# latticeboltzmann/2d-lb

Hardware: AMD Instinct MI355X
Metric: MLUPS (million lattice updates per second), fused D2Q9 BGK step (higher is better)
Workload: dtype f32

## Files before the change

2d-lb_amd/csrc/kernels_deep.h:

```cpp
#pragma once

#ifdef LB_DIAG
#define LB_DEEP_NOCOLLIDE if (!(a.diag & 1))
#else
#define LB_DEEP_NOCOLLIDE
#endif

namespace {

constexpr int DEEP_RW = 1, DEEP_PFD = 1;
constexpr int DEEP_WSLOTS = 8;
constexpr bool deep_pairs(bool mask, int bc) { return !mask && bc == LB_BC_PERIODIC; }

template <int RW, int NL>
struct DeepState {
    Window w[RW > 0 ? RW : 1];
    f4a d0[NL];
    unsigned mhist;
};
typedef unsigned u4v __attribute__((ext_vector_type(4)));
struct DeepCtx {
    int lane, x4, ym, n_iter;
    bool store_lane;
    f4a (*mine)[64], (*other)[64];
    f4a (*ho)[64];
    f4a (*dma)[64];
    unsigned dma_off;
};
constexpr int DEEP_WHOLE = 0, DEEP_FRONT = 1, DEEP_BACK = 2;
constexpr int DEEP_HO_SLOTS = 10;

__device__ __forceinline__ void deep_window_load(f4a (*W)[64], int lane, int it, f4a d0, Window &w)
{
    const int gs = 2 + 3 * (it & 1);
    w.d0 = d0; w.d1 = W[0][lane]; w.d3 = W[1][lane];
    w.g2 = W[gs][lane]; w.g5 = W[gs + 1][lane]; w.g6 = W[gs + 2][lane];
}
template <bool DOWN>
__device__ __forceinline__ void deep_window_push(f4a (*W)[64], int lane, int it, f4a &d0, const f4a (&q)[9])
{
    typedef Dir<DOWN> D_;
    const int gs = 2 + 3 * (it & 1);
    d0 = q[0]; W[0][lane] = q[1]; W[1][lane] = q[3];
    W[gs][lane] = q[D_::A]; W[gs + 1][lane] = q[D_::B]; W[gs + 2][lane] = q[D_::C];
}
template <bool DOWN>
__device__ __forceinline__ void deep_publish(f4a (*W)[64], int lane, int gs, const f4a (&q)[9])
{
    typedef Dir<DOWN> D_;
    W[gs][lane] = q[D_::An]; W[gs + 1][lane] = q[D_::Bn]; W[gs + 2][lane] = q[D_::Cn];
}

constexpr int DEEP_NUM_RECORDS = -1;
__device__ __forceinline__ float *deep_uniform(const float *p)
{
    const unsigned long long v = (unsigned long long)p;
    const unsigned lo = __builtin_amdgcn_readfirstlane((unsigned)v), hi = __builtin_amdgcn_readfirstlane((unsigned)(v >> 32));
    return reinterpret_cast<float *>(((unsigned long long)hi << 32) | lo);
}
__device__ __forceinline__ f4a deep_buf_load(__amdgpu_buffer_rsrc_t r, int vo, int so, int imm)
{
    return __builtin_bit_cast(f4a, __builtin_amdgcn_raw_buffer_load_b128(r, vo + imm, so, 0));
}
template <int BC, bool MASK>
__device__ __forceinline__ void deep_row_load(const StepArgs &a, int r, int x4, Row1 &o)
{
    int ym, yp;
    o.have = step1_rows(a, r, o.rr, ym, yp);
    o.mk = uc4{0, 0, 0, 0};
    o.hsolid = false;
    o.hxc = -1;
    if (o.have) {
        const long long P = a.pitch, S = a.plane;
        const float *s = a.src;
        const int yl = o.rr;
        o.wp = WrapPatch{0.f, 0.f, 0.f, 0.f, 0.f, 0.f};
        if (BC == LB_BC_PERIODIC) {
            const int c = a.nx - 1 - x4;
            const bool wrap_w = x4 == 0, wrap_e = c >= 0 && c < 4;
            if (wrap_w) {
                o.wp.p1 = s[1 * S + (long long)yl * P + a.nx - 1];
                o.wp.p5 = s[5 * S + (long long)ym * P + a.nx - 1];
                o.wp.p8 = s[8 * S + (long long)yp * P + a.nx - 1];
            }
            if (wrap_e) {
                o.wp.w3 = s[3 * S + (long long)yl * P];
                o.wp.w6 = s[6 * S + (long long)ym * P];
                o.wp.w7 = s[7 * S + (long long)yp * P];
            }
        }
        const __amdgpu_buffer_rsrc_t r0 = __builtin_amdgcn_make_buffer_rsrc(deep_uniform(s + (long long)yl * P - 1), 0, DEEP_NUM_RECORDS, 0x00020000);
        const __amdgpu_buffer_rsrc_t rm = __builtin_amdgcn_make_buffer_rsrc(deep_uniform(s + (long long)ym * P - 1), 0, DEEP_NUM_RECORDS, 0x00020000);
        const __amdgpu_buffer_rsrc_t rp = __builtin_amdgcn_make_buffer_rsrc(deep_uniform(s + (long long)yp * P - 1), 0, DEEP_NUM_RECORDS, 0x00020000);
        const unsigned S4 = (unsigned)a.plane * 4u;
        const int vo = x4 * 4;
        o.q[0] = deep_buf_load(r0, vo, 0, 4);
        o.q[1] = deep_buf_load(r0, vo, (int)(S4), 0);
        o.q[2] = deep_buf_load(rm, vo, (int)(2u * S4), 4);
        o.q[3] = deep_buf_load(r0, vo, (int)(3u * S4), 8);
        o.q[4] = deep_buf_load(rp, vo, (int)(4u * S4), 4);
        o.q[5] = deep_buf_load(rm, vo, (int)(5u * S4), 0);
        o.q[6] = deep_buf_load(rm, vo, (int)(6u * S4), 8);
        o.q[7] = deep_buf_load(rp, vo, (int)(7u * S4), 8);
        o.q[8] = deep_buf_load(rp, vo, (int)(8u * S4), 0);
        if (MASK) o.mk = *reinterpret_cast<const uc4 *>(lane_ptr(a.mask + (long long)yl * a.fpitch, x4));
    } else {
        o.wp = WrapPatch{0.f, 0.f, 0.f, 0.f, 0.f, 0.f};
#pragma unroll
        for (int k = 0; k < 9; ++k) o.q[k] = f4a{0.f, 0.f, 0.f, 0.f};
    }
}
#ifdef LB_DIAG
constexpr bool DEEP_MANUAL = false;
#else
constexpr bool DEEP_MANUAL = true;
#endif
__device__ __forceinline__ u4v deep_rsrc_words(const float *p)
{
    const unsigned long long v = (unsigned long long)p;
    return u4v{(unsigned)__builtin_amdgcn_readfirstlane((unsigned)v), (unsigned)__builtin_amdgcn_readfirstlane((unsigned)(v >> 32)), (unsigned)DEEP_NUM_RECORDS,
               0x00020000u};
}
template <int BC, bool MASK>
__device__ __forceinline__ void deep_row_issue(const StepArgs &a, int r, int x4, Row1 &o)
{
    int ym, yp;
    o.have = step1_rows(a, r, o.rr, ym, yp);
    o.hsolid = false;
    o.hxc = -1;
    if (o.have) {
        const long long P = a.pitch, S = a.plane;
        const float *s = a.src;
        const int yl = o.rr;
        if (BC == LB_BC_PERIODIC) {
            const int c = a.nx - 1 - x4;
            const bool wrap_w = x4 == 0, wrap_e = c >= 0 && c < 4;
            if (wrap_w) {
                const float *e = s + a.nx - 1;
                asm volatile("global_load_dword a36, %0, off\n\tglobal_load_dword a37, %1, off\n\tglobal_load_dword a38, %2, off"
                             :: "v"(e + 1 * S + (long long)yl * P), "v"(e + 5 * S + (long long)ym * P), "v"(e + 8 * S + (long long)yp * P)
                             : "memory", "a36", "a37", "a38");
            }
            if (wrap_e) {
                asm volatile("global_load_dword a39, %0, off\n\tglobal_load_dword a40, %1, off\n\tglobal_load_dword a41, %2, off"
                             :: "v"(s + 3 * S + (long long)yl * P), "v"(s + 6 * S + (long long)ym * P), "v"(s + 7 * S + (long long)yp * P)
                             : "memory", "a39", "a40", "a41");
            }
        }
        const u4v r0 = deep_rsrc_words(s + (long long)yl * P - 1), rm = deep_rsrc_words(s + (long long)ym * P - 1),
                  rp = deep_rsrc_words(s + (long long)yp * P - 1);
        const unsigned S4 = (unsigned)a.plane * 4u;
        asm volatile("buffer_load_dwordx4 a[0:3], %0, %1, 0 offen offset:4\n\t"
                     "buffer_load_dwordx4 a[4:7], %0, %1, %4 offen\n\t"
                     "buffer_load_dwordx4 a[8:11], %0, %2, %5 offen offset:4\n\t"
                     "buffer_load_dwordx4 a[12:15], %0, %1, %6 offen offset:8\n\t"
                     "buffer_load_dwordx4 a[16:19], %0, %3, %7 offen offset:4\n\t"
                     "buffer_load_dwordx4 a[20:23], %0, %2, %8 offen\n\t"
                     "buffer_load_dwordx4 a[24:27], %0, %2, %9 offen offset:8\n\t"
                     "buffer_load_dwordx4 a[28:31], %0, %3, %10 offen offset:8\n\t"
                     "buffer_load_dwordx4 a[32:35], %0, %3, %11 offen"
                     :: "v"(x4 * 4), "s"(r0), "s"(rm), "s"(rp), "s"(S4), "s"(2u * S4), "s"(3u * S4), "s"(4u * S4), "s"(5u * S4), "s"(6u * S4),
                        "s"(7u * S4), "s"(8u * S4)
                     : "memory", "a0", "a1", "a2", "a3", "a4", "a5", "a6", "a7", "a8", "a9", "a10", "a11", "a12", "a13",
                       "a14", "a15", "a16", "a17", "a18", "a19", "a20", "a21", "a22", "a23", "a24", "a25", "a26", "a27", "a28",
                       "a29", "a30", "a31", "a32", "a33", "a34", "a35");
        if (MASK) asm volatile("global_load_dword a42, %0, off" :: "v"(lane_ptr(a.mask + (long long)yl * a.fpitch, x4)) : "memory", "a42");
    }
}
template <int BC, bool MASK, int N>
__device__ __forceinline__ void deep_row_take(Row1 &o)
{
    static_assert(N == 0 || N == 9 || N == 12, "the stores of one steady iteration, or nothing");
#define LB_DEEP_TAKE_OUTS "={a[0:3]}"(o.q[0]), "={a[4:7]}"(o.q[1]), "={a[8:11]}"(o.q[2]), "={a[12:15]}"(o.q[3]), \
                          "={a[16:19]}"(o.q[4]), "={a[20:23]}"(o.q[5]), "={a[24:27]}"(o.q[6]), "={a[28:31]}"(o.q[7]), "={a[32:35]}"(o.q[8])
    if (N == 0) asm volatile("s_waitcnt vmcnt(0)" : LB_DEEP_TAKE_OUTS :: "memory");
    else if (N == 9) asm volatile("s_waitcnt vmcnt(9)" : LB_DEEP_TAKE_OUTS :: "memory");
    else asm volatile("s_waitcnt vmcnt(12)" : LB_DEEP_TAKE_OUTS :: "memory");
#undef LB_DEEP_TAKE_OUTS
    o.wp = WrapPatch{0.f, 0.f, 0.f, 0.f, 0.f, 0.f};
    if (BC == LB_BC_PERIODIC)
        asm volatile("" : "={a36}"(o.wp.p1), "={a37}"(o.wp.p5), "={a38}"(o.wp.p8), "={a39}"(o.wp.w3), "={a40}"(o.wp.w6), "={a41}"(o.wp.w7));
    o.mk = uc4{0, 0, 0, 0};
    if (MASK) {
        unsigned m;
        asm volatile("" : "={a42}"(m));
        o.mk = __builtin_bit_cast(uc4, m);
    }
    if (!o.have) {
#pragma unroll
        for (int k = 0; k < 9; ++k) o.q[k] = f4a{0.f, 0.f, 0.f, 0.f};
        o.mk = uc4{0, 0, 0, 0};
    }
}

template <int BC, bool MASK>
__device__ __forceinline__ void deep_row_issue_lds(const StepArgs &a, int r, int x4, unsigned slot, Row1 &o)
{
    int ym, yp;
    o.have = step1_rows(a, r, o.rr, ym, yp);
    o.hsolid = false;
    o.hxc = -1;
    if (o.have) {
        const long long P = a.pitch, S = a.plane;
        const float *s = a.src;
        const int yl = o.rr;
        unsigned m0_kept;
        asm volatile("s_waitcnt lgkmcnt(0)" ::: "memory");
        if (BC == LB_BC_PERIODIC) {
            const int c = a.nx - 1 - x4;
            const bool wrap_w = x4 == 0, wrap_e = c >= 0 && c < 4;
            if (wrap_w) {
                const float *e = s + a.nx - 1;
                asm volatile("s_mov_b32 %0, m0\n\ts_mov_b32 m0, %4\n\ts_nop 0\n\tglobal_load_lds_dword %1, off\n\t"
                             "s_add_u32 m0, m0, 0x100\n\ts_nop 0\n\tglobal_load_lds_dword %2, off\n\t"
                             "s_add_u32 m0, m0, 0x100\n\ts_nop 0\n\tglobal_load_lds_dword %3, off\n\ts_mov_b32 m0, %0"
                             : "=&s"(m0_kept)
                             : "v"(e + 1 * S + (long long)yl * P), "v"(e + 5 * S + (long long)ym * P), "v"(e + 8 * S + (long long)yp * P),
                               "s"(slot + 9 * 1024 + 256)
                             : "memory", "scc");
            }
            if (wrap_e) {
                asm volatile("s_mov_b32 %0, m0\n\ts_mov_b32 m0, %4\n\ts_nop 0\n\tglobal_load_lds_dword %1, off\n\t"
                             "s_add_u32 m0, m0, 0x100\n\ts_nop 0\n\tglobal_load_lds_dword %2, off\n\t"
                             "s_add_u32 m0, m0, 0x100\n\ts_nop 0\n\tglobal_load_lds_dword %3, off\n\ts_mov_b32 m0, %0"
                             : "=&s"(m0_kept)
                             : "v"(s + 3 * S + (long long)yl * P), "v"(s + 6 * S + (long long)ym * P), "v"(s + 7 * S + (long long)yp * P),
                               "s"(slot + 9 * 1024 + 256)
                             : "memory", "scc");
            }
        }
        const u4v r0 = deep_rsrc_words(s + (long long)yl * P - 1), rm = deep_rsrc_words(s + (long long)ym * P - 1),
                  rp = deep_rsrc_words(s + (long long)yp * P - 1);
        const unsigned S4 = (unsigned)a.plane * 4u;
        const int v0 = x4 * 4, v4 = v0 + 4, v8 = v0 + 8;
        asm volatile("s_mov_b32 %0, m0\n\ts_mov_b32 m0, %15\n\ts_nop 0\n\tbuffer_load_dwordx4 %2, %4, 0 offen lds\n\t"
                     "s_add_u32 m0, m0, 0x400\n\ts_nop 0\n\tbuffer_load_dwordx4 %1, %4, %7 offen lds\n\t"
                     "s_add_u32 m0, m0, 0x400\n\ts_nop 0\n\tbuffer_load_dwordx4 %2, %5, %8 offen lds\n\t"
                     "s_add_u32 m0, m0, 0x400\n\ts_nop 0\n\tbuffer_load_dwordx4 %3, %4, %9 offen lds\n\t"
                     "s_add_u32 m0, m0, 0x400\n\ts_nop 0\n\tbuffer_load_dwordx4 %2, %6, %10 offen lds\n\t"
                     "s_add_u32 m0, m0, 0x400\n\ts_nop 0\n\tbuffer_load_dwordx4 %1, %5, %11 offen lds\n\t"
                     "s_add_u32 m0, m0, 0x400\n\ts_nop 0\n\tbuffer_load_dwordx4 %3, %5, %12 offen lds\n\t"
                     "s_add_u32 m0, m0, 0x400\n\ts_nop 0\n\tbuffer_load_dwordx4 %3, %6, %13 offen lds\n\t"
                     "s_add_u32 m0, m0, 0x400\n\ts_nop 0\n\tbuffer_load_dwordx4 %1, %6, %14 offen lds\n\ts_mov_b32 m0, %0"
                     : "=&s"(m0_kept)
                     : "v"(v0), "v"(v4), "v"(v8), "s"(r0), "s"(rm), "s"(rp), "s"(S4), "s"(2u * S4), "s"(3u * S4), "s"(4u * S4), "s"(5u * S4),
                       "s"(6u * S4), "s"(7u * S4), "s"(8u * S4), "s"(slot)
                     : "memory", "scc");
        if (MASK)
            asm volatile("s_mov_b32 %0, m0\n\ts_mov_b32 m0, %2\n\ts_nop 0\n\tglobal_load_lds_dword %1, off\n\ts_mov_b32 m0, %0"
                         : "=&s"(m0_kept) : "v"(lane_ptr(a.mask + (long long)yl * a.fpitch, x4)), "s"(slot + 9 * 1024) : "memory");
    }
}
template <int BC, bool MASK>
__device__ __forceinline__ void deep_row_take_lds(const f4a (*S)[64], int lane, Row1 &o)
{
    asm volatile("s_waitcnt vmcnt(0)" ::: "memory");
    if (o.have) {
#pragma unroll
        for (int k = 0; k < 9; ++k) o.q[k] = S[k][lane];
        const unsigned *X = reinterpret_cast<const unsigned *>(S[9]);
        o.mk = MASK ? __builtin_bit_cast(uc4, X[lane]) : uc4{0, 0, 0, 0};
        o.wp = WrapPatch{0.f, 0.f, 0.f, 0.f, 0.f, 0.f};
        if (BC == LB_BC_PERIODIC) {
            const float e1 = __builtin_bit_cast(float, X[64 + lane]), e2 = __builtin_bit_cast(float, X[128 + lane]),
                        e3 = __builtin_bit_cast(float, X[192 + lane]);
            o.wp = WrapPatch{e1, e2, e3, e1, e2, e3};
        }
    } else {
        o.wp = WrapPatch{0.f, 0.f, 0.f, 0.f, 0.f, 0.f};
#pragma unroll
        for (int k = 0; k < 9; ++k) o.q[k] = f4a{0.f, 0.f, 0.f, 0.f};
        o.mk = uc4{0, 0, 0, 0};
    }
}

__device__ __forceinline__ void deep_row_store(const StepArgs &a, int r, int x4, const f4a (&t)[9])
{
    const __amdgpu_buffer_rsrc_t rd = __builtin_amdgcn_make_buffer_rsrc(deep_uniform(a.dst + (long long)r * a.pitch), 0, DEEP_NUM_RECORDS, 0x00020000);
    const unsigned S4 = (unsigned)a.plane * 4u;
    const int vo = x4 * 4;
    asm volatile("" ::: "memory");
    if (a.nts != 0) {
#pragma unroll
        for (int k = 0; k < 9; ++k) __builtin_amdgcn_raw_buffer_store_b128(__builtin_bit_cast(u4v, t[k]), rd, vo, (int)(k * S4), 2);
    } else {
#pragma unroll
        for (int k = 0; k < 9; ++k) __builtin_amdgcn_raw_buffer_store_b128(__builtin_bit_cast(u4v, t[k]), rd, vo, (int)(k * S4), 0);
    }
}

template <int BC, bool MASK, bool MACRO, int D, int RW, bool DOWN, int NST, int S, int ROLE = DEEP_WHOLE>
__device__ __forceinline__ void deep_stage(const StepArgs &a, const DeepCtx &cx, const int i, const int it,
                                           DeepState<RW, D - 1 - RW> &st, f4a (&qin)[9], f4a &r4, f4a &u4, f4a &v4)
{
    if constexpr (S <= D) {
        constexpr int K = S - 1;
        const int lane = cx.lane, x4 = cx.x4;
        constexpr int L = K > RW ? K - RW - 1 : 0;
        f4a (*W)[64] = cx.mine + L * DEEP_WSLOTS;
        if constexpr (NST >= S) {
            int r, t0_, t1_;
            (void)step1_rows(a, DOWN ? cx.ym - 1 - (i - K) : cx.ym + (i - K), r, t0_, t1_);
            f4a t[9];
            if constexpr (K <= RW) {
                skirt_gather<DOWN>(st.w[K - 1], qin, t);
                window_push_dir<DOWN>(st.w[K - 1], qin);
            } else {
                Window w;
                deep_window_load(W, lane, it, st.d0[L], w);
                skirt_gather<DOWN>(w, qin, t);
                deep_window_push<DOWN>(W, lane, it, st.d0[L], qin);
            }
            LB_DEEP_NOCOLLIDE collide_row<BC, MASK, true>(a, x4, a.y0 + r, t, mask_bits(st.mhist, K), r4, u4, v4);
            if constexpr (S == D && ROLE == DEEP_FRONT) {
#pragma unroll
                for (int k = 0; k < 9; ++k) cx.ho[k][lane] = t[k];
                if (MASK) reinterpret_cast<unsigned *>(cx.ho[9])[lane] = __builtin_bit_cast(unsigned, mask_bits(st.mhist, K));
            } else if constexpr (S == D) {
#ifdef LB_DIAG
                if (!(a.diag & (1 << 22)))
#endif
                if (cx.store_lane) {
                    deep_row_store(a, r, x4, t);
                    if (MACRO) {
                        const long long m = (long long)r * a.fpitch;
                        store_moments(a, m, x4, r4, u4, v4);
                    }
                }
            } else {
                if constexpr (NST == S) {
                    if constexpr (S <= RW) deep_publish<DOWN>(cx.other + (D - 2 - RW) * DEEP_WSLOTS, lane, S == 1 ? 5 : 2, t);
                    else deep_publish<DOWN>(cx.other + (S - RW - 1) * DEEP_WSLOTS, lane, 2 + 3 * (S & 1), t);
                }
                deep_stage<BC, MASK, MACRO, D, RW, DOWN, NST, S + 1, ROLE>(a, cx, i, it, st, t, r4, u4, v4);
            }
        } else if constexpr (NST == S - 1) {
            if constexpr (K <= RW) window_push_dir<DOWN>(st.w[K - 1], qin);
            else deep_window_push<DOWN>(W, lane, it, st.d0[L], qin);
        }
    }
}

template <int BC, bool MASK, bool MACRO, int D, int RW, int PFD, bool DOWN, int NST, int PAR = -1, int ROLE = DEEP_WHOLE>
__device__ __forceinline__ void deep_iter(const StepArgs &a, const DeepCtx &cx, const int i_, DeepState<RW, D - 1 - RW> &st, Row1 &cur,
                                          Row1 &nxt)
{
    static_assert(RW >= 0 && RW <= 2 && D - 1 - RW >= 1 && (ROLE == DEEP_WHOLE ? D - 2 > RW : D - 2 >= RW),
                  "register windows hand over through the last LDS window while it is idle");
    static_assert((D - 1 - RW) * DEEP_WSLOTS <= 40, "a wave has 40 KB of LDS at four waves per CU");
    const int lane = cx.lane, x4 = cx.x4;
    const int i = NST < D ? NST - 1 : i_;
    const int it = PAR >= 0 ? PAR : i;
    auto row_at = [&](int p) { return DOWN ? cx.ym - 1 - p : cx.ym + p; };
    f4a (*MB)[64] = cx.mine + (D - 2 - RW) * DEEP_WSLOTS;
    if (RW >= 1 && NST == 2) { st.w[0].g2 = MB[5][lane]; st.w[0].g5 = MB[6][lane]; st.w[0].g6 = MB[7][lane]; }
    if (RW >= 2 && NST == 3) { st.w[RW >= 2 ? 1 : 0].g2 = MB[2][lane]; st.w[RW >= 2 ? 1 : 0].g5 = MB[3][lane]; st.w[RW >= 2 ? 1 : 0].g6 = MB[4][lane]; }
#ifdef LB_DIAG
    if (!((a.diag & (1 << 23)) && i > 0))
#endif
    if constexpr (ROLE != DEEP_BACK) {
        if (ROLE == DEEP_FRONT) {
            deep_row_take_lds<BC, MASK>(cx.dma, lane, cur);
            deep_row_issue_lds<BC, MASK>(a, row_at(min(i + 1, cx.n_iter - 1)), x4, cx.dma_off, nxt);
        } else if (PFD && DEEP_MANUAL) {
            deep_row_take<BC, MASK, (NST < D ? 0 : (MACRO ? 12 : 9))>(cur);
            deep_row_issue<BC, MASK>(a, row_at(min(i + 1, cx.n_iter - 1)), x4, nxt);
        } else {
            static_assert(PFD == 1 || ROLE == DEEP_BACK, "a march that gathers its rows gathers them one ahead");
            deep_row_load<BC, MASK>(a, row_at(min(i + 1, cx.n_iter - 1)), x4, nxt);
        }
    }
    f4a (&q1)[9] = cur.q;
    f4a r4, u4, v4;
    const uc4 mk = cur.mk;
    if (ROLE != DEEP_BACK && cur.have) {
        gather_merge<BC, true>(a, x4, q1, cur.wp);
        LB_DEEP_NOCOLLIDE collide_row<BC, MASK, true>(a, x4, a.y0 + cur.rr, q1, mk, r4, u4, v4);
    }
    if (NST == 1) {
        if constexpr (RW >= 1) deep_publish<DOWN>(cx.other + (D - 2 - RW) * DEEP_WSLOTS, lane, 5, q1);
        else deep_publish<DOWN>(cx.other, lane, 2 + 3 * 1, q1);
    }
    deep_stage<BC, MASK, MACRO, D, RW, DOWN, NST, 2, ROLE>(a, cx, i, it, st, q1, r4, u4, v4);
    if (MASK) st.mhist = ((st.mhist | mask_word(mk)) << 1) & (0x01010101u * (unsigned)(((1 << D) - 2) & 0xff));
    if (ROLE == DEEP_WHOLE && NST < D) __syncthreads();
}

template <int BC, bool MASK, bool MACRO, int D, int RW, int PFD, bool DOWN, int NST>
__device__ __forceinline__ void deep_fill(const StepArgs &a, const DeepCtx &cx, DeepState<RW, D - 1 - RW> &st, Row1 &ra, Row1 &rb)
{
    if constexpr (NST < D) {
        if ((NST & 1) == 0) deep_iter<BC, MASK, MACRO, D, RW, PFD, DOWN, NST>(a, cx, NST - 1, st, rb, ra);
        else deep_iter<BC, MASK, MACRO, D, RW, PFD, DOWN, NST>(a, cx, NST - 1, st, ra, rb);
        deep_fill<BC, MASK, MACRO, D, RW, PFD, DOWN, NST + 1>(a, cx, st, ra, rb);
    }
}

template <int BC, bool MASK, bool MACRO, int D, int RW, int PFD, bool DOWN>
__device__ __forceinline__ void deep_march(const StepArgs &a, const int x0, const int ym, const int len, f4a (*mine)[64],
                                           f4a (*other)[64])
{
    DeepCtx cx;
    cx.lane = threadIdx.x;
    const int xr = x0 + cx.lane * 4;
    cx.x4 = skirt_column<BC>(a, xr, deep_skirt_lanes(D));
    cx.store_lane = skirt_store_lane(a, cx.lane, xr, deep_skirt_lanes(D));
    cx.ym = ym; cx.n_iter = len + D - 1;
    cx.mine = mine; cx.other = other;
    DeepState<RW, D - 1 - RW> st = {};
    auto row_at = [&](int p) { return DOWN ? ym - 1 - p : ym + p; };
    static_assert(PFD == 1, "a whole march gathers one row ahead");
    Row1 ra, rb;
    if (DEEP_MANUAL) deep_row_issue<BC, MASK>(a, row_at(0), cx.x4, ra);
    else deep_row_load<BC, MASK>(a, row_at(0), cx.x4, ra);
    deep_fill<BC, MASK, MACRO, D, RW, PFD, DOWN, 1>(a, cx, st, ra, rb);
    if (DEEP_MANUAL) asm volatile("s_waitcnt vmcnt(0)" ::: "memory");
    if (!deep_pairs(MASK, BC)) {
        if ((D - 1) & 1) ra = rb;
        for (int i = D - 1; i < cx.n_iter; ++i) {
            deep_iter<BC, MASK, MACRO, D, RW, PFD, DOWN, D>(a, cx, i, st, ra, rb);
            ra = rb;
        }
    } else {
        constexpr int P0 = (D - 1) & 1;
        int i = D - 1;
        for (; i + 1 < cx.n_iter; i += 2) {
            deep_iter<BC, MASK, MACRO, D, RW, PFD, DOWN, D, P0>(a, cx, i, st, P0 ? rb : ra, P0 ? ra : rb);
            deep_iter<BC, MASK, MACRO, D, RW, PFD, DOWN, D, 1 - P0>(a, cx, i + 1, st, P0 ? ra : rb, P0 ? rb : ra);
        }
        if (i < cx.n_iter) deep_iter<BC, MASK, MACRO, D, RW, PFD, DOWN, D, P0>(a, cx, i, st, P0 ? rb : ra, P0 ? ra : rb);
    }
    if (DEEP_MANUAL) asm volatile("s_waitcnt vmcnt(0)" ::: "memory");
}

template <int BC, bool MASK, bool MACRO, int D, int RW, int PFD>
__global__ __launch_bounds__(64 * STEP4_WAVES, PFD ? 1 : 2) void k_deep(const StepArgs a, int strips, int seg_rows, int nsegs, int row_end)
{
    __shared__ f4a lds_win[STEP4_WAVES][(D - 1 - RW) * DEEP_WSLOTS][64];
    const int wy = __builtin_amdgcn_readfirstlane(threadIdx.y);
    const int item = xcd_item(blockIdx.x, gridDim.x);
#ifdef LB_DIAG
    const unsigned long long diag_t0 = __builtin_amdgcn_s_memrealtime();
#endif
    int sx, sy;
    if (item < strips * nsegs) {
        sx = item % strips;
        sy = item / strips;
    } else {
        if (!a.edge_seg_rows) return;
        const int j = item - strips * nsegs;
        sx = (j & 1) ? strips - 1 : 0;
        sy = nsegs + (j >> 1);
    }
    int stride = a.seg_stride;
    if (a.edge_seg_rows && (sx == 0 || sx == strips - 1)) stride = seg_rows = a.edge_seg_rows;
    const int ya = a.row_begin + sy * stride;
    if (ya >= row_end) return;
    const int yb = min(ya + seg_rows, row_end);
    const int ym = ya + (yb - ya) / 2;
    const int x0 = sx * deep_valid(D) - 4 * deep_skirt_lanes(D);
    if (wy == 0) deep_march<BC, MASK, MACRO, D, RW, PFD, true>(a, x0, ym, ym - ya, lds_win[0], lds_win[1]);
    else deep_march<BC, MASK, MACRO, D, RW, PFD, false>(a, x0, ym, yb - ym, lds_win[1], lds_win[0]);
#ifdef LB_DIAG
    if ((a.diag & 4096) && threadIdx.x == 0) {
        __builtin_amdgcn_s_waitcnt(0);
        const unsigned long long t1 = __builtin_amdgcn_s_memrealtime();
        unsigned *o = reinterpret_cast<unsigned *>(a.rho) + 8 * (item * STEP4_WAVES + wy);
        o[0] = (unsigned)diag_t0; o[1] = (unsigned)(diag_t0 >> 32); o[2] = (unsigned)t1; o[3] = (unsigned)(t1 >> 32);
        o[4] = __builtin_amdgcn_s_getreg((31 << 11) | 20);
        o[5] = __builtin_amdgcn_s_getreg((31 << 11) | 4);
        o[6] = (unsigned)(item * STEP4_WAVES + wy); o[7] = (unsigned)(wy ? yb - ym : ym - ya);
    }
#endif
}

}
```

2d-lb_amd/csrc/kernels_step5.h:

```cpp
#pragma once

namespace {


struct March5State {
    Window w1, w2;
    unsigned mhist;
};
struct March5Ctx {
    int lane, x4, ym, n_iter, wy;
    bool store_lane;
    unsigned slot;
    f4a (*W3)[64], (*W4)[64], (*P3)[64], (*P4)[64];
    f4a (*R2)[64], (*Q2)[64];
};

__device__ __forceinline__ float wave_from_left(float v)
{
    const int i = __builtin_bit_cast(int, v);
    return __builtin_bit_cast(float, __builtin_amdgcn_update_dpp(0, i, 0x138, 0xf, 0xf, true));
}
__device__ __forceinline__ float wave_from_right(float v)
{
    const int i = __builtin_bit_cast(int, v);
    return __builtin_bit_cast(float, __builtin_amdgcn_update_dpp(0, i, 0x130, 0xf, 0xf, true));
}
__device__ __forceinline__ f4a skirt_left(f4a v) { return f4a{wave_from_left(v.w), v.x, v.y, v.z}; }
__device__ __forceinline__ f4a skirt_right(f4a v) { return f4a{v.y, v.z, v.w, wave_from_right(v.x)}; }
template <bool DOWN>
__device__ __forceinline__ void skirt_gather(const Window &w, const f4a (&q)[9], f4a (&t)[9])
{
    typedef Dir<DOWN> D;
    t[0] = w.d0;
    t[1] = skirt_left(w.d1);
    t[3] = skirt_right(w.d3);
    t[D::A] = w.g2;
    t[D::B] = skirt_left(w.g5);
    t[D::C] = skirt_right(w.g6);
    t[D::An] = q[D::An];
    t[D::Cn] = skirt_right(q[D::Cn]);
    t[D::Bn] = skirt_left(q[D::Bn]);
}

template <int BC, bool MASK, bool MACRO, bool PF, bool DOWN, int NST>
__device__ __forceinline__ void march5_iter(const StepArgs &a, const March5Ctx &cx, const int i_, March5State &st, Row1 &cur)
{
    const int lane = cx.lane, x4 = cx.x4;
    const long long S = a.plane;
    const int i = NST < 5 ? NST - 1 : i_;
    const int it = i;
    auto row_at = [&](int p) { return DOWN ? cx.ym - 1 - p : cx.ym + p; };
    f4a(*W3)[64] = cx.W3;
    f4a(*W4)[64] = cx.W4;
    Window &w1 = st.w1, &w2 = st.w2;

    prio_turn(a, i, cx.slot);
    if (NST == 2) { w1.g2 = W4[6][lane]; w1.g5 = W4[7][lane]; w1.g6 = W4[8][lane]; }
    if (NST == 3 && !PF) { w2.g2 = W4[3][lane]; w2.g5 = W4[4][lane]; w2.g6 = W4[5][lane]; }
    if (!PF) row1_load<BC, MASK>(a, row_at(i), x4, false, 0, cur);
    f4a (&q1)[9] = cur.q;
    f4a r4, u4, v4;
    const uc4 mk = cur.mk;
    if (cur.have) {
        gather_merge<BC, true>(a, x4, q1, cur.wp);
        collide_row<BC, MASK>(a, x4, a.y0 + cur.rr, q1, mk, r4, u4, v4);
    }
    const int r_next = row_at(min(i + 1, cx.n_iter - 1));
    if (NST == 1) lds_publish<DOWN>(cx.P4, lane, 6, q1);
    f4a q2[9];
    if (NST >= 2) {
        int r2, t0_, t1_;
        (void)step1_rows(a, row_at(i - 1), r2, t0_, t1_);
        skirt_gather<DOWN>(w1, q1, q2);
        window_push_dir<DOWN>(w1, q1);
        if (PF) row1_load<BC, MASK>(a, r_next, x4, false, 0, cur);
        collide_row<BC, MASK>(a, x4, a.y0 + r2, q2, mask_bits(st.mhist, 1), r4, u4, v4);
        if (NST == 2) {
            if (PF) lds_publish<DOWN>(cx.Q2, lane, 0, q2);
            else lds_publish<DOWN>(cx.P4, lane, 3, q2);
        }
    } else {
        window_push_dir<DOWN>(w1, q1);
        if (PF) row1_load<BC, MASK>(a, r_next, x4, false, 0, cur);
    }
    f4a q3[9];
    if (NST >= 3) {
        int r3, t0_, t1_;
        (void)step1_rows(a, row_at(i - 2), r3, t0_, t1_);
        if (PF) {
            typedef Dir<DOWN> D;
            const int gs = 3 * (it & 1);
            w2.g2 = cx.R2[gs][lane]; w2.g5 = cx.R2[gs + 1][lane]; w2.g6 = cx.R2[gs + 2][lane];
            skirt_gather<DOWN>(w2, q2, q3);
            cx.R2[gs][lane] = q2[D::A]; cx.R2[gs + 1][lane] = q2[D::B]; cx.R2[gs + 2][lane] = q2[D::C];
            w2.d0 = q2[0]; w2.d1 = q2[1]; w2.d3 = q2[3];
        } else {
            skirt_gather<DOWN>(w2, q2, q3);
            window_push_dir<DOWN>(w2, q2);
        }
        collide_row<BC, MASK>(a, x4, a.y0 + r3, q3, mask_bits(st.mhist, 2), r4, u4, v4);
        if (NST == 3) lds_publish<DOWN>(cx.P3, lane, 6, q3);
    } else if (NST == 2) {
        if (PF) {
            typedef Dir<DOWN> D;
            cx.R2[3][lane] = q2[D::A]; cx.R2[4][lane] = q2[D::B]; cx.R2[5][lane] = q2[D::C];
            w2.d0 = q2[0]; w2.d1 = q2[1]; w2.d3 = q2[3];
        } else {
            window_push_dir<DOWN>(w2, q2);
        }
    }
    f4a q4[9];
    if (NST >= 4) {
        int r4_, t0_, t1_;
        (void)step1_rows(a, row_at(i - 3), r4_, t0_, t1_);
        Window w3;
        lds_window_load(W3, lane, it, w3);
        skirt_gather<DOWN>(w3, q3, q4);
        lds_window_push<DOWN>(W3, lane, it, q3);
        collide_row<BC, MASK>(a, x4, a.y0 + r4_, q4, mask_bits(st.mhist, 3), r4, u4, v4);
        if (NST == 4) lds_publish<DOWN>(cx.P4, lane, 3, q4);
    } else if (NST == 3) {
        lds_window_push<DOWN>(W3, lane, it, q3);
    }
    if (NST >= 5) {
        int r5, t0_, t1_;
        (void)step1_rows(a, row_at(i - 4), r5, t0_, t1_);
        Window w4;
        lds_window_load(W4, lane, it, w4);
        f4a t[9];
        skirt_gather<DOWN>(w4, q4, t);
        lds_window_push<DOWN>(W4, lane, it, q4);
        collide_row<BC, MASK>(a, x4, a.y0 + r5, t, mask_bits(st.mhist, 4), r4, u4, v4);
        if (cx.store_lane) {
            const long long o = (long long)r5 * a.pitch;
            float *d = a.dst + o;
            store_row9(a.nts != 0, d, S, x4, t);
            if (MACRO) {
                const long long m = (long long)r5 * a.fpitch;
                store_moments(a, m, x4, r4, u4, v4);
            }
        }
    } else if (NST == 4) {
        lds_window_push<DOWN>(W4, lane, it, q4);
    }
    if (MASK) st.mhist = ((st.mhist | mask_word(mk)) << 1) & 0x1e1e1e1eu;
    if (NST < 5) __syncthreads();
}

template <int BC>
__device__ __forceinline__ int skirt_column(const StepArgs &a, int xr, int skl)
{
    if (BC == LB_BC_PERIODIC) return xr < 0 ? xr + a.nx : (xr >= a.nx ? (xr - a.nx < 4 * skl ? xr - a.nx : 4 * (skl - 1)) : xr);
    return min(max(xr, 0), (a.nx - 1) & ~3);
}
__device__ __forceinline__ bool skirt_store_lane(const StepArgs &a, int lane, int xr, int skl)
{
    return lane >= skl && lane <= 63 - skl && xr < a.nx;
}

template <int BC, bool MASK, bool MACRO, bool PF, bool DOWN>
__device__ __forceinline__ void march5(const StepArgs &a, const int x0, const int ym, const int len, const int wy,
                                       f4a (*mine)[64], f4a (*other)[64], const unsigned slot)
{
    March5Ctx cx;
    cx.lane = threadIdx.x;
    const int xr = x0 + cx.lane * 4;
    cx.x4 = skirt_column<BC>(a, xr, STEP5_SKIRT / 4);
    cx.store_lane = skirt_store_lane(a, cx.lane, xr, STEP5_SKIRT / 4);
    cx.ym = ym; cx.n_iter = len + 4; cx.wy = wy; cx.slot = slot;
    cx.W3 = mine; cx.W4 = mine + 9; cx.R2 = mine + 18;
    cx.P3 = other; cx.P4 = other + 9; cx.Q2 = other + 18;
    March5State st = {};
    auto row_at = [&](int p) { return DOWN ? ym - 1 - p : ym + p; };
    Row1 cur;
    if (PF) row1_load<BC, MASK>(a, row_at(0), cx.x4, false, 0, cur);
    march5_iter<BC, MASK, MACRO, PF, DOWN, 1>(a, cx, 0, st, cur);
    march5_iter<BC, MASK, MACRO, PF, DOWN, 2>(a, cx, 1, st, cur);
    march5_iter<BC, MASK, MACRO, PF, DOWN, 3>(a, cx, 2, st, cur);
    march5_iter<BC, MASK, MACRO, PF, DOWN, 4>(a, cx, 3, st, cur);
    for (int i = 4; i < cx.n_iter; ++i) march5_iter<BC, MASK, MACRO, PF, DOWN, 5>(a, cx, i, st, cur);
}

template <int BC, bool MASK, bool MACRO, bool PF>
__global__ __launch_bounds__(64 * STEP4_WAVES, 2) void k_step5(const StepArgs a, int strips, int seg_rows, int nsegs, int row_end)
{
    __shared__ f4a lds_win[STEP4_WAVES][PF ? 24 : 18][64];
    const int wy = __builtin_amdgcn_readfirstlane(threadIdx.y);
    const int item = xcd_item(blockIdx.x, gridDim.x);
    const unsigned slot = __builtin_amdgcn_s_getreg((4 << 11) | 4) & 1u;
    int sx, sy;
    if (item < strips * nsegs) {
        sx = item % strips;
        sy = item / strips;
    } else {
        if (!a.edge_seg_rows) return;
        const int j = item - strips * nsegs;
        sx = (j & 1) ? strips - 1 : 0;
        sy = nsegs + (j >> 1);
    }
    int stride = a.seg_stride;
    if (a.edge_seg_rows && (sx == 0 || sx == strips - 1)) stride = seg_rows = a.edge_seg_rows;
    const int ya = a.row_begin + sy * stride;
    if (ya >= row_end) return;
    const int yb = min(ya + seg_rows, row_end);
    const int ym = ya + (yb - ya) / 2;
    const int x0 = sx * STEP5_VALID - STEP5_SKIRT;
    if (wy == 0) march5<BC, MASK, MACRO, PF, true>(a, x0, ym, ym - ya, 0, lds_win[0], lds_win[1], slot);
    else march5<BC, MASK, MACRO, PF, false>(a, x0, ym, yb - ym, 1, lds_win[1], lds_win[0], slot);
}

}
```

Measured before the change: 505,900.

## Store LDS window slots pre-shifted so deep stages skip cross-lane skirt shifts

Left- and right-shifted window slots in the deep march are now stored in LDS in a component-planar layout. The neighbour-lane shift is folded into the store addresses, so the later load returns values that are already shifted. This removes the skirt_left/skirt_right cross-lane operations (DPP or permute) on the gather path, at the cost of scalar-dword LDS stores and loads in place of 128-bit ones. Register-window mailbox publishes keep the old layout. The second LDS window base is now computed from a scalar offset hidden behind an asm barrier.

```diff
diff --git a/2d-lb_amd/csrc/kernels_deep.h b/2d-lb_amd/csrc/kernels_deep.h
--- a/2d-lb_amd/csrc/kernels_deep.h
+++ b/2d-lb_amd/csrc/kernels_deep.h
@@ -1,4 +1,6 @@
 #pragma once
+
+#include "window_slots.h"
 
 #ifdef LB_DIAG
 #define LB_DEEP_NOCOLLIDE if (!(a.diag & 1))
@@ -30,22 +32,42 @@
 constexpr int DEEP_WHOLE = 0, DEEP_FRONT = 1, DEEP_BACK = 2;
 constexpr int DEEP_HO_SLOTS = 10;
 
+template <int KIND>
+__device__ __forceinline__ f4a wslot_load(const f4a (*W)[64], int slot, int lane)
+{
+    const float *F = reinterpret_cast<const float *>(W[slot]);
+    return f4a{F[wslot_load_dword(KIND, lane, 0)], F[wslot_load_dword(KIND, lane, 1)], F[wslot_load_dword(KIND, lane, 2)],
+               F[wslot_load_dword(KIND, lane, 3)]};
+}
+template <int KIND>
+__device__ __forceinline__ void wslot_store(f4a (*W)[64], int slot, int lane, f4a v)
+{
+    float *F = reinterpret_cast<float *>(W[slot]);
+    F[wslot_store_dword(KIND, lane, 0)] = v.x; F[wslot_store_dword(KIND, lane, 1)] = v.y;
+    F[wslot_store_dword(KIND, lane, 2)] = v.z; F[wslot_store_dword(KIND, lane, 3)] = v.w;
+}
 __device__ __forceinline__ void deep_window_load(f4a (*W)[64], int lane, int it, f4a d0, Window &w)
 {
     const int gs = 2 + 3 * (it & 1);
-    w.d0 = d0; w.d1 = W[0][lane]; w.d3 = W[1][lane];
-    w.g2 = W[gs][lane]; w.g5 = W[gs + 1][lane]; w.g6 = W[gs + 2][lane];
+    w.d0 = d0; w.d1 = wslot_load<WSLOT_LEFT>(W, 0, lane); w.d3 = wslot_load<WSLOT_RIGHT>(W, 1, lane);
+    w.g2 = W[gs][lane]; w.g5 = wslot_load<WSLOT_LEFT>(W, gs + 1, lane); w.g6 = wslot_load<WSLOT_RIGHT>(W, gs + 2, lane);
 }
 template <bool DOWN>
 __device__ __forceinline__ void deep_window_push(f4a (*W)[64], int lane, int it, f4a &d0, const f4a (&q)[9])
 {
     typedef Dir<DOWN> D_;
     const int gs = 2 + 3 * (it & 1);
-    d0 = q[0]; W[0][lane] = q[1]; W[1][lane] = q[3];
-    W[gs][lane] = q[D_::A]; W[gs + 1][lane] = q[D_::B]; W[gs + 2][lane] = q[D_::C];
+    d0 = q[0]; wslot_store<WSLOT_LEFT>(W, 0, lane, q[1]); wslot_store<WSLOT_RIGHT>(W, 1, lane, q[3]);
+    W[gs][lane] = q[D_::A]; wslot_store<WSLOT_LEFT>(W, gs + 1, lane, q[D_::B]); wslot_store<WSLOT_RIGHT>(W, gs + 2, lane, q[D_::C]);
 }
 template <bool DOWN>
 __device__ __forceinline__ void deep_publish(f4a (*W)[64], int lane, int gs, const f4a (&q)[9])
+{
+    typedef Dir<DOWN> D_;
+    W[gs][lane] = q[D_::An]; wslot_store<WSLOT_LEFT>(W, gs + 1, lane, q[D_::Bn]); wslot_store<WSLOT_RIGHT>(W, gs + 2, lane, q[D_::Cn]);
+}
+template <bool DOWN>
+__device__ __forceinline__ void deep_publish_mailbox(f4a (*W)[64], int lane, int gs, const f4a (&q)[9])
 {
     typedef Dir<DOWN> D_;
     W[gs][lane] = q[D_::An]; W[gs + 1][lane] = q[D_::Bn]; W[gs + 2][lane] = q[D_::Cn];
@@ -308,7 +330,7 @@
             } else {
                 Window w;
                 deep_window_load(W, lane, it, st.d0[L], w);
-                skirt_gather<DOWN>(w, qin, t);
+                skirt_gather_shifted<DOWN>(w, qin, t);
                 deep_window_push<DOWN>(W, lane, it, st.d0[L], qin);
             }
             LB_DEEP_NOCOLLIDE collide_row<BC, MASK, true>(a, x4, a.y0 + r, t, mask_bits(st.mhist, K), r4, u4, v4);
@@ -329,7 +351,7 @@
                 }
             } else {
                 if constexpr (NST == S) {
-                    if constexpr (S <= RW) deep_publish<DOWN>(cx.other + (D - 2 - RW) * DEEP_WSLOTS, lane, S == 1 ? 5 : 2, t);
+                    if constexpr (S <= RW) deep_publish_mailbox<DOWN>(cx.other + (D - 2 - RW) * DEEP_WSLOTS, lane, S == 1 ? 5 : 2, t);
                     else deep_publish<DOWN>(cx.other + (S - RW - 1) * DEEP_WSLOTS, lane, 2 + 3 * (S & 1), t);
                 }
                 deep_stage<BC, MASK, MACRO, D, RW, DOWN, NST, S + 1, ROLE>(a, cx, i, it, st, t, r4, u4, v4);
@@ -378,7 +400,7 @@
         LB_DEEP_NOCOLLIDE collide_row<BC, MASK, true>(a, x4, a.y0 + cur.rr, q1, mk, r4, u4, v4);
     }
     if (NST == 1) {
-        if constexpr (RW >= 1) deep_publish<DOWN>(cx.other + (D - 2 - RW) * DEEP_WSLOTS, lane, 5, q1);
+        if constexpr (RW >= 1) deep_publish_mailbox<DOWN>(cx.other + (D - 2 - RW) * DEEP_WSLOTS, lane, 5, q1);
         else deep_publish<DOWN>(cx.other, lane, 2 + 3 * 1, q1);
     }
     deep_stage<BC, MASK, MACRO, D, RW, DOWN, NST, 2, ROLE>(a, cx, i, it, st, q1, r4, u4, v4);
@@ -459,8 +481,10 @@
     const int yb = min(ya + seg_rows, row_end);
     const int ym = ya + (yb - ya) / 2;
     const int x0 = sx * deep_valid(D) - 4 * deep_skirt_lanes(D);
-    if (wy == 0) deep_march<BC, MASK, MACRO, D, RW, PFD, true>(a, x0, ym, ym - ya, lds_win[0], lds_win[1]);
-    else deep_march<BC, MASK, MACRO, D, RW, PFD, false>(a, x0, ym, yb - ym, lds_win[1], lds_win[0]);
+    int win1 = (D - 1 - RW) * DEEP_WSLOTS;
+    asm volatile("" : "+s"(win1));
+    if (wy == 0) deep_march<BC, MASK, MACRO, D, RW, PFD, true>(a, x0, ym, ym - ya, lds_win[0], lds_win[0] + win1);
+    else deep_march<BC, MASK, MACRO, D, RW, PFD, false>(a, x0, ym, yb - ym, lds_win[0] + win1, lds_win[0]);
 #ifdef LB_DIAG
     if ((a.diag & 4096) && threadIdx.x == 0) {
         __builtin_amdgcn_s_waitcnt(0);
diff --git a/2d-lb_amd/csrc/kernels_step5.h b/2d-lb_amd/csrc/kernels_step5.h
--- a/2d-lb_amd/csrc/kernels_step5.h
+++ b/2d-lb_amd/csrc/kernels_step5.h
@@ -37,6 +37,20 @@
     t[D::A] = w.g2;
     t[D::B] = skirt_left(w.g5);
     t[D::C] = skirt_right(w.g6);
+    t[D::An] = q[D::An];
+    t[D::Cn] = skirt_right(q[D::Cn]);
+    t[D::Bn] = skirt_left(q[D::Bn]);
+}
+template <bool DOWN>
+__device__ __forceinline__ void skirt_gather_shifted(const Window &w, const f4a (&q)[9], f4a (&t)[9])
+{
+    typedef Dir<DOWN> D;
+    t[0] = w.d0;
+    t[1] = w.d1;
+    t[3] = w.d3;
+    t[D::A] = w.g2;
+    t[D::B] = w.g5;
+    t[D::C] = w.g6;
     t[D::An] = q[D::An];
     t[D::Cn] = skirt_right(q[D::Cn]);
     t[D::Bn] = skirt_left(q[D::Bn]);
diff --git a/2d-lb_amd/csrc/window_slots.h b/2d-lb_amd/csrc/window_slots.h
--- /dev/null
+++ b/2d-lb_amd/csrc/window_slots.h
@@ -0,0 +1,12 @@
+#pragma once
+
+constexpr int WSLOT_LANES = 64, WSLOT_DWORDS = 256;
+constexpr int WSLOT_LANE = 0, WSLOT_LEFT = 1, WSLOT_RIGHT = 2;
+
+constexpr int wslot_store_dword(int kind, int lane, int c)
+{
+    if (kind == WSLOT_LEFT) return c == 3 ? ((lane + 1) & (WSLOT_LANES - 1)) : WSLOT_LANES * (c + 1) + lane;
+    if (kind == WSLOT_RIGHT) return c == 0 ? WSLOT_LANES * 3 + ((lane - 1) & (WSLOT_LANES - 1)) : WSLOT_LANES * (c - 1) + lane;
+    return 4 * lane + c;
+}
+constexpr int wslot_load_dword(int kind, int lane, int j) { return kind == WSLOT_LANE ? 4 * lane + j : WSLOT_LANES * j + lane; }
```

New measurement: 508,600 (median of 6 runs). Within noise of the previous version (+0.5%).
